# azrael417/mlperf-deepcam

Measured on AMD Instinct MI355X. Metric: samples/sec (768x1152x16) train step, higher is better.
Workload: dtype bf16; 1 GPU; DeepLabV3+/Xception train step (fwd + weighted CE + bwd + LAMB), 768x1152x16, local_batch=8, bf16 activations / fp32 master weights, random-init seed 333; local_batch=8, global_batch=8, parallelism=dp1, optimizer=LAMB, hip_graph=False, launch_list_replay=False

## Files before the change

### mlperf-deepcam_amd/csrc/common.h

```cpp
#pragma once
#include <hip/hip_runtime.h>
#include <stdint.h>

#include <mutex>

#include "../../include/deepcam_hip.h"

namespace dc {

typedef __bf16 bf16;
typedef __attribute__((ext_vector_type(8))) __bf16 bf16x8;
typedef __attribute__((ext_vector_type(4))) __bf16 bf16x4;
typedef __attribute__((ext_vector_type(4))) short short4v;
typedef __attribute__((ext_vector_type(4))) float f32x4;
typedef __attribute__((ext_vector_type(2))) float f32x2;

struct alignas(16) vec16 {
  uint32_t w[4];
};

template <typename T>
struct Elem;
template <>
struct Elem<float> {
  static constexpr int kPerVec = 4;
  static constexpr int kDtype = DC_F32;
  __device__ static inline float load(const float* p) { return *p; }
  __device__ static inline void store(float* p, float v) { *p = v; }
};
template <>
struct Elem<bf16> {
  static constexpr int kPerVec = 8;
  static constexpr int kDtype = DC_BF16;
  __device__ static inline float load(const bf16* p) { return (float)*p; }
  __device__ static inline void store(bf16* p, float v) { *p = (bf16)v; }
};

__device__ inline void unpack(const vec16& v, float (&f)[4], float) {
#pragma unroll
  for (int i = 0; i < 4; ++i) f[i] = __uint_as_float(v.w[i]);
}
__device__ inline void unpack(const vec16& v, float (&f)[8], bf16) {
#pragma unroll
  for (int i = 0; i < 4; ++i) {
    f[2 * i] = __uint_as_float(v.w[i] << 16);
    f[2 * i + 1] = __uint_as_float(v.w[i] & 0xffff0000u);
  }
}
__device__ inline uint32_t pack2_bf16(float lo, float hi) {
  typedef __attribute__((ext_vector_type(2))) __bf16 bf16x2;
  bf16x2 r;
  r[0] = (bf16)lo;
  r[1] = (bf16)hi;
  return __builtin_bit_cast(uint32_t, r);
}
__device__ inline void pack(vec16& v, const float (&f)[4], float) {
#pragma unroll
  for (int i = 0; i < 4; ++i) v.w[i] = __float_as_uint(f[i]);
}
__device__ inline void pack(vec16& v, const float (&f)[8], bf16) {
#pragma unroll
  for (int i = 0; i < 4; ++i) v.w[i] = pack2_bf16(f[2 * i], f[2 * i + 1]);
}

__device__ inline vec16 zero16() {
  vec16 z;
  z.w[0] = z.w[1] = z.w[2] = z.w[3] = 0u;
  return z;
}
__device__ inline vec16 ldg16(const void* p) { return *reinterpret_cast<const vec16*>(p); }
__device__ inline void stg16(void* p, const vec16& v) { *reinterpret_cast<vec16*>(p) = v; }

__device__ inline float wave_sum(float v) {
#pragma unroll
  for (int o = 32; o > 0; o >>= 1) v += __shfl_xor(v, o, 64);
  return v;
}
__device__ inline double wave_sum(double v) {
#pragma unroll
  for (int o = 32; o > 0; o >>= 1) v += __shfl_xor(v, o, 64);
  return v;
}

inline int cdiv(long a, long b) { return (int)((a + b - 1) / b); }

struct Options {
  int igemm256 = 1;
  int igemm256p = 1;
  int igemm256p_wgs = 0;
  int igemm256p_min = 257;
  int igemm256_splitk = 1;
  int pw384 = 1;
  int pw224 = 1;
  int pw192 = 1;
  int thin_tile = 1;
  int wgrad384 = 1;
  int wgrad384_slots = 192;
  int wgrad384_min_stages = 96;
  int head_fused = 1;
  int head_dgrad_fused = 1;
  int head_wgrad_fused = 1;
  int dw_tile = 1;
  int dw_wgrad_tpb = 0;
  int dw_pipe = 1;
  int bn_apply_rows = 1;
};
extern Options g_options;

const void* zero_page(hipError_t* err);

}

#define DC_ONCE(...)                               \
  do {                                             \
    static std::once_flag once_flag__;             \
    std::call_once(once_flag__, [&] { __VA_ARGS__; }); \
  } while (0)

namespace dc {
extern thread_local bool g_launch_log_on;
void launch_log_note(const char* name);
}

#define DC_LAUNCHED(name)                                  \
  do {                                                     \
    hipError_t e__ = hipGetLastError();                    \
    if (e__ != hipSuccess) return dc_set_error(e__, __FILE__, __LINE__); \
    if (dc::g_launch_log_on) dc::launch_log_note(name);    \
  } while (0)
#define DC_CHECK_LAUNCH() DC_LAUNCHED("aux")

extern "C" int dc_set_error(int code, const char* file, int line);
extern "C" int dc_fail(const char* msg, const char* file, int line);
extern "C" int dc_check_view(const void* ptr, int ld, int c, int dtype, const char* what);
#define DC_REQUIRE(cond, msg)                                  \
  do {                                                         \
    if (!(cond)) return dc_fail(msg, __FILE__, __LINE__);      \
  } while (0)
```

### mlperf-deepcam_amd/csrc/dwtile.hip

```cpp
#include "common.h"
#include "dwtile.h"
#include "dwtile_common.h"
#include "bn_fin.h"
#include "mfma_tile.h"

namespace dc {

constexpr int DT_TH = 8;

template <int DIL, int CG>
struct TileCfg {
  static constexpr int TH = DT_TH, TW = 8 * (32 / CG);
  static constexpr int HH = TH + 2 * DIL, HW = TW + 2 * DIL, HP = HH * HW;
  static constexpr int ITER = (HP * CG + 255) / 256;
  static constexpr int LDS_BYTES = ITER * 256 * 16;
  static constexpr int NSL = 128 / CG;
  static constexpr int SPR = TW / DT_PX;
  static constexpr int SPT = TH * SPR / NSL;
  static_assert(SPT * NSL == TH * SPR, "tile does not divide into strips");
};

static __device__ __attribute__((aligned(256))) unsigned char dwt_zero_page[256];

template <typename T, int DIL, int CG>
__device__ inline void stage_halo(char* smem, const T* __restrict__ in, int ldin, int n, int y0, int x0, int cg0, int ngroups, int H,
                                  int W) {
  typedef TileCfg<DIL, CG> K;
  constexpr int KPV = Elem<T>::kPerVec;
  const int tid = threadIdx.x;
  const int wv = __builtin_amdgcn_readfirstlane(tid >> 6);
  const int g = tid % CG;
  const bool gok = cg0 + g < ngroups;
  const T* base = in + (size_t)n * H * W * ldin + (size_t)(cg0 + g) * KPV;
#pragma unroll
  for (int it = 0; it < K::ITER; ++it) {
    const int hp = (it * 256 + tid) / CG;
    const int hy = hp / K::HW, hx = hp - hy * K::HW;
    const int iy = y0 - DIL + hy, ix = x0 - DIL + hx;
    const bool ok = gok && hp < K::HP && (unsigned)iy < (unsigned)H && (unsigned)ix < (unsigned)W;
    const void* src = ok ? (const void*)(base + ((size_t)iy * W + ix) * ldin) : (const void*)dwt_zero_page;
    __builtin_amdgcn_global_load_lds((gas_ptr)src, (lds_ptr)(smem + (it * 256 + wv * 64) * 16), 16, 0, 0);
  }
}

template <typename T, int DIL, bool FLIP, int CG, bool WG = false, int FIN = 0>
__global__ __launch_bounds__(256) void dwt_kernel(const T* __restrict__ in, int ldin, const float* __restrict__ wp,
                                                  const T* __restrict__ addend, int ldadd, T* __restrict__ out, int ldout, int H, int W,
                                                  int C, int ncgb, int ntx, int nty, const float* __restrict__ pscale,
                                                  const float* __restrict__ pshift, int prelu, const DwBnStats st, const BnFinArgs fin) {
  typedef TileCfg<DIL, CG> K;
  constexpr int KPV = Elem<T>::kPerVec, KH = KPV / 2;
  constexpr int WC = DT_PX + 2 * DIL;
  extern __shared__ __attribute__((aligned(16))) char smem[];
  const int t = xcd_remap(blockIdx.x, gridDim.x);
  const int cgb = t % ncgb;
  const int tile_id = t / ncgb;
  int r = t / ncgb;
  const int tx = r % ntx;
  r /= ntx;
  const int ty = r % nty, n = r / nty;
  const int ngroups = C / KPV;
  const int cg0 = cgb * CG, y0 = ty * K::TH, x0 = tx * K::TW;
  stage_halo<T, DIL, CG>(smem, in, ldin, n, y0, x0, cg0, ngroups, H, W);

  const int h = threadIdx.x % (2 * CG), sl = threadIdx.x / (2 * CG);
  const bool cok = cg0 + (h >> 1) < ngroups;
  const int ch0 = cok ? cg0 * KPV + h * KH : 0;
  float wk[9][KH];
  load_taps<KH>(wp, ch0, C, FLIP, wk);
  const float* ps = pscale;
  const float* psh = pshift;
  int cbase = 0;
  float fsc = 0.f, fsh = 0.f;
  if constexpr (FIN == 2) {
    constexpr int CW = CG * KPV;
    if (threadIdx.x < CW) {
      const int c = cg0 * KPV + threadIdx.x;
      if (c < C) {
        double s, q;
        sum_row_load(fin.slab, C, c, s, q);
        bn_fin_coefs(fin, c, s, q, tile_id == 0, fsc, fsh);
      }
    }
    if (t == 0 && threadIdx.x == 0 && fin.nbt != nullptr) *fin.nbt += 1;
  }
  if constexpr (FIN == 1) {
    constexpr int CW = CG * KPV;
    __shared__ float fincoef[2][CW];
    __shared__ double finred[2][4][CW];
    {
      double s, q;
      slab_quad_sum2<CW>(fin.slab, fin.rows, C, cg0 * KPV, finred, s, q);
      if (threadIdx.x < CW) {
        const int c = cg0 * KPV + threadIdx.x;
        float sc = 0.f, sh = 0.f;
        if (c < C) bn_fin_coefs(fin, c, s, q, tile_id == 0, sc, sh);
        fincoef[0][threadIdx.x] = sc;
        fincoef[1][threadIdx.x] = sh;
      }
      if (t == 0 && threadIdx.x == 0 && fin.nbt != nullptr) *fin.nbt += 1;
      ps = fincoef[0];
      psh = fincoef[1];
      cbase = cg0 * KPV;
    }
  }
  __syncthreads();
  if constexpr (FIN == 2) {
    constexpr int CW = CG * KPV;
    constexpr bool SLACK = K::LDS_BYTES - K::HP * CG * 16 >= 2 * CW * (int)sizeof(float);
    float* coef;
    if constexpr (SLACK) {
      coef = reinterpret_cast<float*>(smem + K::LDS_BYTES) - 2 * CW;
    } else {
      __shared__ float fincoef2[2 * CW];
      coef = fincoef2;
    }
    if (threadIdx.x < CW) {
      coef[threadIdx.x] = fsc;
      coef[CW + threadIdx.x] = fsh;
    }
    __syncthreads();
    ps = coef;
    psh = coef + CW;
    cbase = cg0 * KPV;
  }
  if (!FLIP && ps != nullptr) {
    bn_transform_tile<T, K::HH, K::HW, CG>(smem, y0 - DIL, x0 - DIL, H, W, ps, psh, prelu, cg0, ngroups, cbase);
    __syncthreads();
  }
  const bool stats = FLIP && st.slab != nullptr;
  if (!cok && !stats && !WG) return;
  BnAcc<KH> bn;
  if (stats) bn.init(st, ch0);
  else if (WG) bn.init_affine(st, ch0);
  float dwa[WG ? 9 : 1][KH];
  if constexpr (WG) {
#pragma unroll
    for (int t9 = 0; t9 < 9; ++t9)
#pragma unroll
      for (int e = 0; e < KH; ++e) dwa[t9][e] = 0.f;
  }

  const char* tile = smem + h * 8;
#pragma unroll 1
  for (int k = 0; k < (cok ? K::SPT : 0); ++k) {
    const int q = sl + K::NSL * k;
    const int row = q / K::SPR, xs = (q % K::SPR) * DT_PX;
    const int oy = y0 + row;
    vec8 yv[DT_PX];
    if (stats || WG) {
#pragma unroll
      for (int j = 0; j < DT_PX; ++j) {
        const int ox = x0 + xs + j;
        vec8 z;
        z.w[0] = z.w[1] = 0u;
        yv[j] = (oy < H && ox < W) ? *reinterpret_cast<const vec8*>(reinterpret_cast<const T*>(st.y) + (((size_t)n * H + oy) * W + ox) * st.ldy + ch0) : z;
      }
    }
    vec8 av[DT_PX];
    if (FLIP && addend != nullptr) {
#pragma unroll
      for (int j = 0; j < DT_PX; ++j) {
        const int ox = x0 + xs + j;
        vec8 z;
        z.w[0] = z.w[1] = 0u;
        av[j] = (oy < H && ox < W) ? *reinterpret_cast<const vec8*>(addend + (((size_t)n * H + oy) * W + ox) * ldadd + ch0) : z;
      }
    }
    float acc[DT_PX][KH];
#pragma unroll
    for (int j = 0; j < DT_PX; ++j)
#pragma unroll
      for (int e = 0; e < KH; ++e) acc[j][e] = 0.f;
    float xh[WG ? DT_PX : 1][KH];
    if constexpr (WG) {
#pragma unroll
      for (int j = 0; j < DT_PX; ++j) {
        const bool in = oy < H && x0 + xs + j < W;
        float yf[KH];
        unpack8(yv[j], yf, T());
#pragma unroll
        for (int e = 0; e < KH; ++e) {
          const float v = fmaf(yf[e], bn.ms[e], bn.mh[e]);
          yf[e] = st.relu ? fmaxf(v, 0.f) : v;
        }
        vec8 r;
        pack8(r, yf, T());
        unpack8(r, xh[j], T());
        if (!in) {
#pragma unroll
          for (int e = 0; e < KH; ++e) xh[j][e] = 0.f;
        }
      }
    }
#pragma unroll
    for (int ky = 0; ky < 3; ++ky) {
#pragma unroll
      for (int c = 0; c < WC; ++c) {
        float f[KH];
        unpack8(*reinterpret_cast<const vec8*>(tile + ((row + ky * DIL) * K::HW + xs + c) * (CG * 16)), f, T());
#pragma unroll
        for (int kx = 0; kx < 3; ++kx) {
          const int j = c - kx * DIL;
          if (j >= 0 && j < DT_PX) {
#pragma unroll
            for (int e = 0; e < KH; ++e) acc[j][e] = fmaf(f[e], wk[ky * 3 + kx][e], acc[j][e]);
            if constexpr (WG) {
#pragma unroll
              for (int e = 0; e < KH; ++e) dwa[8 - (ky * 3 + kx)][e] = fmaf(f[e], xh[j][e], dwa[8 - (ky * 3 + kx)][e]);
            }
          }
        }
      }
    }
    if (oy < H) {
#pragma unroll
      for (int j = 0; j < DT_PX; ++j) {
        const int ox = x0 + xs + j;
        if (ox < W) {
          const size_t opix = ((size_t)n * H + oy) * W + ox;
          if (FLIP && addend != nullptr) {
            float a[KH];
            unpack8(av[j], a, T());
#pragma unroll
            for (int e = 0; e < KH; ++e) acc[j][e] += a[e];
          }
          vec8 v;
          pack8(v, acc[j], T());
          *reinterpret_cast<vec8*>(out + opix * ldout + ch0) = v;
          if (stats) {
            float gs[KH], yf[KH];
            unpack8(v, gs, T());
            unpack8(yv[j], yf, T());
            bn.add(gs, yf, st.relu);
          }
        }
      }
    }
  }
  if (stats) {
    __syncthreads();
    bn_acc_store<KH, K::NSL, CG * KPV>(reinterpret_cast<float*>(smem), bn.a, bn.b, cok, h, sl, st, tile_id, cg0 * KPV, C);
  }
  if constexpr (WG) {
    __syncthreads();
    float* red = reinterpret_cast<float*>(smem);
    constexpr int CW = CG * KPV;
    if (cok) {
#pragma unroll
      for (int tp = 0; tp < 9; ++tp)
#pragma unroll
        for (int e = 0; e < KH; ++e) red[(sl * 9 + tp) * CW + h * KH + e] = dwa[tp][e];
    }
    __syncthreads();
    for (int i = threadIdx.x; i < 9 * CW; i += 256) {
      const int tp = i / CW, cl = i % CW;
      const int c = cg0 * KPV + cl;
      if (c < C) {
        float sacc = 0.f;
#pragma unroll
        for (int qq = 0; qq < K::NSL; ++qq) sacc += red[(qq * 9 + tp) * CW + cl];
        st.wslab[((size_t)tile_id * 9 + tp) * C + c] = sacc;
      }
    }
  }
}

template <typename T, int DIL, int CG>
__global__ __launch_bounds__(256) void dwt_wgrad_kernel(const T* __restrict__ x, int ldx, const T* __restrict__ dy, int lddy,
                                                        float* __restrict__ slab, int H, int W, int C, int ncgb, int ntx, int nty,
                                                        int ntiles, int tpb, const float* __restrict__ pscale,
                                                        const float* __restrict__ pshift, int prelu) {
  typedef TileCfg<DIL, CG> K;
  constexpr int KPV = Elem<T>::kPerVec, KH = KPV / 2;
  constexpr int WC = DT_PX + 2 * DIL;
  extern __shared__ __attribute__((aligned(16))) char smem[];
  const int t = xcd_remap(blockIdx.x, gridDim.x);
  const int cgb = t % ncgb, srow = t / ncgb;
  const int ngroups = C / KPV;
  const int cg0 = cgb * CG;
  const int h = threadIdx.x % (2 * CG), sl = threadIdx.x / (2 * CG);
  const bool cok = cg0 + (h >> 1) < ngroups;
  const int ch0 = cok ? cg0 * KPV + h * KH : 0;
  float acc[9][KH];
#pragma unroll
  for (int tp = 0; tp < 9; ++tp)
#pragma unroll
    for (int e = 0; e < KH; ++e) acc[tp][e] = 0.f;

  const int tbeg = srow * tpb, tend = min(ntiles, tbeg + tpb);
  const char* tile = smem + h * 8;
  for (int ti = tbeg; ti < tend; ++ti) {
    const int tx = ti % ntx;
    int r = ti / ntx;
    const int ty = r % nty, n = r / nty;
    const int y0 = ty * K::TH, x0 = tx * K::TW;
    if (ti != tbeg) __syncthreads();
    stage_halo<T, DIL, CG>(smem, x, ldx, n, y0, x0, cg0, ngroups, H, W);
    auto load_dy = [&](int k, vec8 (&gv)[DT_PX]) {
      const int q = sl + K::NSL * k;
      const int row = q / K::SPR, xs = (q % K::SPR) * DT_PX;
      const int oy = y0 + row;
#pragma unroll
      for (int j = 0; j < DT_PX; ++j) {
        const int ox = x0 + xs + j;
        const bool ok = cok && oy < H && ox < W;
        vec8 z;
        z.w[0] = z.w[1] = 0u;
        gv[j] = ok ? *reinterpret_cast<const vec8*>(dy + (((size_t)n * H + oy) * W + ox) * lddy + ch0) : z;
      }
    };
    vec8 gcur[DT_PX], gnext[DT_PX];
    load_dy(0, gcur);
    __syncthreads();
    if (pscale != nullptr) {
      bn_transform_tile<T, K::HH, K::HW, CG>(smem, y0 - DIL, x0 - DIL, H, W, pscale, pshift, prelu, cg0, ngroups);
      __syncthreads();
    }
    if (cok) {
#pragma unroll 1
      for (int k = 0; k < K::SPT; ++k) {
        if (k + 1 < K::SPT) load_dy(k + 1, gnext);
        const int q = sl + K::NSL * k;
        const int row = q / K::SPR, xs = (q % K::SPR) * DT_PX;
        float gf[DT_PX][KH];
#pragma unroll
        for (int j = 0; j < DT_PX; ++j) unpack8(gcur[j], gf[j], T());
#pragma unroll
        for (int ky = 0; ky < 3; ++ky)
#pragma unroll
          for (int c = 0; c < WC; ++c) {
            float f[KH];
            unpack8(*reinterpret_cast<const vec8*>(tile + ((row + ky * DIL) * K::HW + xs + c) * (CG * 16)), f, T());
#pragma unroll
            for (int kx = 0; kx < 3; ++kx) {
              const int j = c - kx * DIL;
              if (j >= 0 && j < DT_PX) {
#pragma unroll
                for (int e = 0; e < KH; ++e) acc[ky * 3 + kx][e] = fmaf(gf[j][e], f[e], acc[ky * 3 + kx][e]);
              }
            }
          }
#pragma unroll
        for (int j = 0; j < DT_PX; ++j) gcur[j] = gnext[j];
      }
    }
  }
  __syncthreads();
  float* red = reinterpret_cast<float*>(smem);
  constexpr int CW = CG * KPV;
#pragma unroll
  for (int tp = 0; tp < 9; ++tp)
#pragma unroll
    for (int e = 0; e < KH; ++e) red[(sl * 9 + tp) * CW + h * KH + e] = acc[tp][e];
  __syncthreads();
  for (int i = threadIdx.x; i < 9 * CW; i += 256) {
    const int tp = i / CW, cl = i % CW;
    const int c = cg0 * KPV + cl;
    if (c < C) {
      float s = 0.f;
#pragma unroll
      for (int q = 0; q < K::NSL; ++q) s += red[(q * 9 + tp) * CW + cl];
      slab[((size_t)srow * 9 + tp) * C + c] = s;
    }
  }
}

__global__ __launch_bounds__(256) void dwt_reduce_kernel(const float* __restrict__ slab, float* __restrict__ grad, int rows, int C) {
  __shared__ double red[16][16];
  const int cl = threadIdx.x & 15, rl = threadIdx.x >> 4;
  const int n = 9 * C;
  const int i = blockIdx.x * 16 + cl;
  double a0 = 0.0, a1 = 0.0;
  if (i < n) {
    int r = rl;
    for (; r + 16 < rows; r += 32) {
      a0 += (double)slab[(size_t)r * n + i];
      a1 += (double)slab[(size_t)(r + 16) * n + i];
    }
    if (r < rows) a0 += (double)slab[(size_t)r * n + i];
  }
  red[rl][cl] = a0 + a1;
  __syncthreads();
  if (threadIdx.x < 16 && blockIdx.x * 16 + threadIdx.x < n) {
    const int j = blockIdx.x * 16 + threadIdx.x;
    double s = 0.0;
#pragma unroll
    for (int k = 0; k < 16; ++k) s += red[k][threadIdx.x];
    const int tp = j / C, c = j % C;
    grad[(size_t)c * 9 + tp] = (float)s;
  }
}

int dw_tile_reduce(const float* slab, float* grad_w, int rows, int C, hipStream_t st) {
  hipLaunchKernelGGL(dwt_reduce_kernel, dim3(cdiv(9 * C, 16)), dim3(256), 0, st, slab, grad_w, rows, C);
  DC_LAUNCHED("dw_tile_reduce");
  return 0;
}

static int pick_cg(int ngroups) { return ngroups <= 8 ? 8 : ngroups <= 16 ? 16 : 32; }

struct TileGrid {
  int cg, ncgb, ntx, nty, ntiles;
};
static TileGrid tile_grid(int ngroups, int N, int H, int W) {
  TileGrid t;
  t.cg = pick_cg(ngroups);
  const int tw = 8 * (32 / t.cg);
  t.ncgb = cdiv(ngroups, t.cg);
  t.ntx = cdiv(W, tw);
  t.nty = cdiv(H, DT_TH);
  t.ntiles = N * t.ntx * t.nty;
  return t;
}

static int wgrad_tpb(const TileGrid& t) {
  if (g_options.dw_wgrad_tpb > 0) return g_options.dw_wgrad_tpb;
  long tpb = ((long)t.ntiles * t.ncgb + 256) / 512;
  if (tpb < 1) tpb = 1;
  while (cdiv(t.ntiles, tpb) > DWT_MAX_ROWS) ++tpb;
  return (int)tpb;
}

int dw_tile_rows(int dtype, int C, int N, int H, int W) { return tile_grid(C / (dtype == DC_BF16 ? 8 : 4), N, H, W).ntiles; }

size_t dw_tile_wgrad_workspace(int C, int N, int H, int W) {
  size_t best = 0;
  for (int kpv = 4; kpv <= 8; kpv += 4) {
    if (C % kpv) continue;
    const TileGrid t = tile_grid(C / kpv, N, H, W);
    const int rows = t.ntiles < DWT_MAX_ROWS ? t.ntiles : DWT_MAX_ROWS;
    const size_t b = (size_t)rows * 9 * C * sizeof(float);
    if (b > best) best = b;
  }
  return best;
}

template <typename T, int DIL, bool FLIP, int CG>
static void launch_fwd1(const TileGrid& t, const void* in, int ldin, const float* wp, const void* addend, int ldadd, void* out,
                        int ldout, int H, int W, int C, hipStream_t st, const float* pscale, const float* pshift, int prelu, const DwBnStats& bs, const BnFinArgs& fin) {
  if constexpr (FLIP) {
    if (bs.wslab != nullptr) {
      constexpr int FOLD = TileCfg<DIL, CG>::NSL * 9 * CG * Elem<T>::kPerVec * (int)sizeof(float);
      constexpr int LDSW = TileCfg<DIL, CG>::LDS_BYTES > FOLD ? TileCfg<DIL, CG>::LDS_BYTES : FOLD;
      DC_ONCE((void)hipFuncSetAttribute(reinterpret_cast<const void*>(&dwt_kernel<T, DIL, true, CG, true>), hipFuncAttributeMaxDynamicSharedMemorySize, LDSW));
      hipLaunchKernelGGL((dwt_kernel<T, DIL, true, CG, true>), dim3(t.ntiles * t.ncgb), dim3(256), LDSW, st, (const T*)in, ldin, wp,
                         (const T*)addend, ldadd, (T*)out, ldout, H, W, C, t.ncgb, t.ntx, t.nty, pscale, pshift, prelu, bs, fin);
      return;
    }
  }
  constexpr int LDS = TileCfg<DIL, CG>::LDS_BYTES;
  if constexpr (!FLIP) {
    if (fin.slab != nullptr && fin.rows == SUM_ROW) {
      DC_ONCE((void)hipFuncSetAttribute(reinterpret_cast<const void*>(&dwt_kernel<T, DIL, false, CG, false, 2>), hipFuncAttributeMaxDynamicSharedMemorySize, LDS));
      hipLaunchKernelGGL((dwt_kernel<T, DIL, false, CG, false, 2>), dim3(t.ntiles * t.ncgb), dim3(256), LDS, st, (const T*)in, ldin, wp,
                         (const T*)addend, ldadd, (T*)out, ldout, H, W, C, t.ncgb, t.ntx, t.nty, pscale, pshift, prelu, bs, fin);
      return;
    }
    if (fin.slab != nullptr) {
      DC_ONCE((void)hipFuncSetAttribute(reinterpret_cast<const void*>(&dwt_kernel<T, DIL, false, CG, false, 1>), hipFuncAttributeMaxDynamicSharedMemorySize, LDS));
      hipLaunchKernelGGL((dwt_kernel<T, DIL, false, CG, false, 1>), dim3(t.ntiles * t.ncgb), dim3(256), LDS, st, (const T*)in, ldin, wp,
                         (const T*)addend, ldadd, (T*)out, ldout, H, W, C, t.ncgb, t.ntx, t.nty, pscale, pshift, prelu, bs, fin);
      return;
    }
  }
  DC_ONCE((void)hipFuncSetAttribute(reinterpret_cast<const void*>(&dwt_kernel<T, DIL, FLIP, CG>), hipFuncAttributeMaxDynamicSharedMemorySize, LDS));
  hipLaunchKernelGGL((dwt_kernel<T, DIL, FLIP, CG>), dim3(t.ntiles * t.ncgb), dim3(256), LDS, st, (const T*)in, ldin, wp,
                     (const T*)addend, ldadd, (T*)out, ldout, H, W, C, t.ncgb, t.ntx, t.nty, pscale, pshift, prelu, bs, fin);
}

template <typename T, int DIL, bool FLIP>
static void launch_fwd2(const TileGrid& t, const void* in, int ldin, const float* wp, const void* addend, int ldadd, void* out,
                        int ldout, int H, int W, int C, hipStream_t st, const float* pscale, const float* pshift, int prelu, const DwBnStats& bs, const BnFinArgs& fin) {
  if (t.cg == 32) launch_fwd1<T, DIL, FLIP, 32>(t, in, ldin, wp, addend, ldadd, out, ldout, H, W, C, st, pscale, pshift, prelu, bs, fin);
  else if (t.cg == 16) launch_fwd1<T, DIL, FLIP, 16>(t, in, ldin, wp, addend, ldadd, out, ldout, H, W, C, st, pscale, pshift, prelu, bs, fin);
  else launch_fwd1<T, DIL, FLIP, 8>(t, in, ldin, wp, addend, ldadd, out, ldout, H, W, C, st, pscale, pshift, prelu, bs, fin);
}

int launch_dw_tile(int dtype, int dil, bool flip, const void* in, int ldin, const float* wp, const void* addend, int ldadd,
                   void* out, int ldout, int N, int H, int W, int C, hipStream_t st, const float* pscale, const float* pshift, int prelu,
                   const DwBnStats* bnstats, const BnFinArgs* finp) {
  const int kpv = dtype == DC_BF16 ? 8 : 4;
  BnFinArgs fin;
  if (finp != nullptr) fin = *finp; else fin.slab = nullptr;
  DC_REQUIRE(finp == nullptr || (!flip && !dw_pipe_forward() && finp->rows <= FIN_RL && finp->parts == 0),
             "dc_dwconv_fwd_fin: a forward pass on the tiled kernel over a slab of at most dc_bn_bwd_apply_fin_max_rows() rows");
  if ((flip || dw_pipe_forward()) && (long)N * H * W < (1L << 31) && dw_pipe_rows(dtype, C, dil, N, H, W) > 0)
    return launch_dw_pipe(dil, flip, in, ldin, wp, addend, ldadd, out, ldout, N, H, W, C, st, pscale, pshift, prelu, bnstats);
  DC_REQUIRE(bnstats == nullptr || bnstats->rows != SUM_ROW, "dc_dwconv_dgrad_*_sum: a sum row is served by the pipelined kernel only (dc_dwconv_dgrad_sum_row_ok)");
  const TileGrid t = tile_grid(C / kpv, N, H, W);
  DC_REQUIRE((long)t.ntiles * t.ncgb < (1L << 31) && (long)N * H * W < (1L << 31), "dc_dwconv: tensor too large for the tiled path");
  DwBnStats bs;
  if (bnstats != nullptr) bs = *bnstats; else { bs.slab = nullptr; bs.y = nullptr; bs.ldy = 0; bs.mean = bs.invstd = bs.mscale = bs.mshift = nullptr; bs.relu = 0; bs.rows = 0; bs.wslab = nullptr; }
  if (bs.slab != nullptr) bs.rows = t.ntiles;
#define DWT(TT, D, F) launch_fwd2<TT, D, F>(t, in, ldin, wp, addend, ldadd, out, ldout, H, W, C, st, pscale, pshift, prelu, bs, fin)
  if (dtype == DC_BF16) {
    if (dil == 1) { if (flip) DWT(bf16, 1, true); else DWT(bf16, 1, false); }
    else          { if (flip) DWT(bf16, 2, true); else DWT(bf16, 2, false); }
  } else {
    if (dil == 1) { if (flip) DWT(float, 1, true); else DWT(float, 1, false); }
    else          { if (flip) DWT(float, 2, true); else DWT(float, 2, false); }
  }
#undef DWT
  DC_LAUNCHED(flip ? "dw_tile_dgrad" : "dw_tile_fwd");
  return 0;
}

template <typename T, int DIL, int CG>
static void launch_wg1(const TileGrid& t, int tpb, int rows, const void* x, int ldx, const void* dy, int lddy, float* slab, int H,
                       int W, int C, hipStream_t st, const float* pscale, const float* pshift, int prelu) {
  constexpr int FOLD = TileCfg<DIL, CG>::NSL * 9 * CG * Elem<T>::kPerVec * (int)sizeof(float);
  constexpr int LDS = TileCfg<DIL, CG>::LDS_BYTES > FOLD ? TileCfg<DIL, CG>::LDS_BYTES : FOLD;
  DC_ONCE((void)hipFuncSetAttribute(reinterpret_cast<const void*>(&dwt_wgrad_kernel<T, DIL, CG>), hipFuncAttributeMaxDynamicSharedMemorySize, LDS));
  hipLaunchKernelGGL((dwt_wgrad_kernel<T, DIL, CG>), dim3(rows * t.ncgb), dim3(256), LDS, st, (const T*)x, ldx, (const T*)dy, lddy,
                     slab, H, W, C, t.ncgb, t.ntx, t.nty, t.ntiles, tpb, pscale, pshift, prelu);
}

template <typename T, int DIL>
static void launch_wg2(const TileGrid& t, int tpb, int rows, const void* x, int ldx, const void* dy, int lddy, float* slab, int H,
                       int W, int C, hipStream_t st, const float* pscale, const float* pshift, int prelu) {
  if (t.cg == 32) launch_wg1<T, DIL, 32>(t, tpb, rows, x, ldx, dy, lddy, slab, H, W, C, st, pscale, pshift, prelu);
  else if (t.cg == 16) launch_wg1<T, DIL, 16>(t, tpb, rows, x, ldx, dy, lddy, slab, H, W, C, st, pscale, pshift, prelu);
  else launch_wg1<T, DIL, 8>(t, tpb, rows, x, ldx, dy, lddy, slab, H, W, C, st, pscale, pshift, prelu);
}

int launch_dw_tile_wgrad(int dtype, int dil, const void* x, int ldx, const void* dy, int lddy, float* slab, float* grad_w, int N,
                         int H, int W, int C, hipStream_t st, const float* pscale, const float* pshift, int prelu) {
  const int kpv = dtype == DC_BF16 ? 8 : 4;
  const TileGrid t = tile_grid(C / kpv, N, H, W);
  const int tpb = wgrad_tpb(t);
  const int rows = cdiv(t.ntiles, tpb);
  DC_REQUIRE(rows <= DWT_MAX_ROWS, "dc_dwconv_wgrad: tiles-per-workgroup override needs more slab rows than the workspace holds");
  DC_REQUIRE((long)N * H * W < (1L << 31), "dc_dwconv_wgrad: tensor too large for the tiled path");
  if (dtype == DC_BF16) {
    if (dil == 1) launch_wg2<bf16, 1>(t, tpb, rows, x, ldx, dy, lddy, slab, H, W, C, st, pscale, pshift, prelu);
    else launch_wg2<bf16, 2>(t, tpb, rows, x, ldx, dy, lddy, slab, H, W, C, st, pscale, pshift, prelu);
  } else {
    if (dil == 1) launch_wg2<float, 1>(t, tpb, rows, x, ldx, dy, lddy, slab, H, W, C, st, pscale, pshift, prelu);
    else launch_wg2<float, 2>(t, tpb, rows, x, ldx, dy, lddy, slab, H, W, C, st, pscale, pshift, prelu);
  }
  DC_LAUNCHED("dw_tile_wgrad");
  hipLaunchKernelGGL(dwt_reduce_kernel, dim3(cdiv(9 * C, 16)), dim3(256), 0, st, (const float*)slab, grad_w, rows, C);
  DC_LAUNCHED("dw_tile_reduce");
  return 0;
}

}
```

### mlperf-deepcam_amd/csrc/dwtile_common.h

```cpp
#pragma once
#include "common.h"

namespace dc {

constexpr int DT_PX = 4;

__device__ inline int xcd_remap(int bid, int nwg) {
  const int q8 = nwg >> 3, r8 = nwg & 7, xcd = bid & 7, slot = bid >> 3;
  return (xcd < r8 ? xcd * (q8 + 1) : r8 * (q8 + 1) + (xcd - r8) * q8) + slot;
}

struct alignas(8) vec8 {
  uint32_t w[2];
};
__device__ inline void unpack8(const vec8& v, float (&f)[2], float) {
  f[0] = __uint_as_float(v.w[0]);
  f[1] = __uint_as_float(v.w[1]);
}
__device__ inline void unpack8(const vec8& v, float (&f)[4], bf16) {
#pragma unroll
  for (int i = 0; i < 2; ++i) {
    f[2 * i] = __uint_as_float(v.w[i] << 16);
    f[2 * i + 1] = __uint_as_float(v.w[i] & 0xffff0000u);
  }
}
__device__ inline void pack8(vec8& v, const float (&f)[2], float) {
  v.w[0] = __float_as_uint(f[0]);
  v.w[1] = __float_as_uint(f[1]);
}
__device__ inline void pack8(vec8& v, const float (&f)[4], bf16) {
  v.w[0] = pack2_bf16(f[0], f[1]);
  v.w[1] = pack2_bf16(f[2], f[3]);
}

template <int KH>
__device__ inline void load_taps(const float* __restrict__ wp, int ch0, int C, bool flip, float (&wk)[9][KH]) {
#pragma unroll
  for (int t = 0; t < 9; ++t) {
    const float* src = wp + (size_t)(flip ? 8 - t : t) * C + ch0;
    if constexpr (KH == 4) {
      const float4 v = *reinterpret_cast<const float4*>(src);
      wk[t][0] = v.x; wk[t][1] = v.y; wk[t][2] = v.z; wk[t][3] = v.w;
    } else {
      const float2 v = *reinterpret_cast<const float2*>(src);
      wk[t][0] = v.x; wk[t][1] = v.y;
    }
  }
}


struct DwBnStats {
  const void* y;
  int ldy;
  const float* mean;
  const float* invstd;
  const float* mscale;
  const float* mshift;
  int relu;
  float* slab;
  int rows;
  float* wslab;
};

template <int KH>
struct BnAcc {
  float mu[KH], is[KH], ms[KH], mh[KH], a[KH], b[KH];
  __device__ inline void init(const DwBnStats& st, int ch0) {
    const bool affine = st.relu || st.wslab != nullptr;
#pragma unroll
    for (int e = 0; e < KH; ++e) {
      mu[e] = st.mean[ch0 + e];
      is[e] = st.invstd[ch0 + e];
      ms[e] = affine ? st.mscale[ch0 + e] : 0.f;
      mh[e] = affine ? st.mshift[ch0 + e] : 0.f;
      a[e] = b[e] = 0.f;
    }
  }
  __device__ inline void init_affine(const DwBnStats& st, int ch0) {
#pragma unroll
    for (int e = 0; e < KH; ++e) {
      mu[e] = is[e] = a[e] = b[e] = 0.f;
      ms[e] = st.mscale != nullptr ? st.mscale[ch0 + e] : 1.f;
      mh[e] = st.mshift != nullptr ? st.mshift[ch0 + e] : 0.f;
    }
  }
  __device__ inline void add(const float (&g)[KH], const float (&yv)[KH], int relu) {
#pragma unroll
    for (int e = 0; e < KH; ++e) {
      const float gm = (!relu || fmaf(yv[e], ms[e], mh[e]) > 0.f) ? g[e] : 0.f;
      a[e] += gm;
      b[e] = fmaf(gm, (yv[e] - mu[e]) * is[e], b[e]);
    }
  }
};

template <int KH, int NSL, int CW>
__device__ inline void bn_acc_store(float* red, const float (&a)[KH], const float (&b)[KH], bool cok, int h, int sl, const DwBnStats& st,
                                    int tile, int c_base, int C) {
  if (cok) {
#pragma unroll
    for (int e = 0; e < KH; ++e) {
      red[(sl * 2 + 0) * CW + h * KH + e] = a[e];
      red[(sl * 2 + 1) * CW + h * KH + e] = b[e];
    }
  }
  __syncthreads();
  for (int i = threadIdx.x; i < 2 * CW; i += 256) {
    const int which = i / CW, cl = i % CW;
    if (c_base + cl < C) {
      float s = 0.f;
#pragma unroll
      for (int q = 0; q < NSL; ++q) s += red[(q * 2 + which) * CW + cl];
      st.slab[((size_t)which * st.rows + tile) * C + c_base + cl] = s;
    }
  }
}

template <typename T, int HH, int HW, int CG>
__device__ inline void bn_transform_tile(char* smem, int iy0, int ix0, int H, int W, const float* __restrict__ pscale,
                                         const float* __restrict__ pshift, int prelu, int cg0, int ngroups, int cbase = 0) {
  constexpr int KPV = Elem<T>::kPerVec;
  constexpr int HP = HH * HW, ITER = (HP * CG + 255) / 256;
  const int tid = threadIdx.x, g = tid % CG;
  if (cg0 + g >= ngroups) return;
  float sc[KPV], sh[KPV];
#pragma unroll
  for (int e = 0; e < KPV; ++e) {
    sc[e] = pscale[(cg0 + g) * KPV + e - cbase];
    sh[e] = pshift[(cg0 + g) * KPV + e - cbase];
  }
#pragma unroll 2
  for (int it = 0; it < ITER; ++it) {
    const int slot = it * 256 + tid;
    const int hp = slot / CG;
    const int hy = hp / HW, hx = hp - hy * HW;
    const int iy = iy0 + hy, ix = ix0 + hx;
    if (hp < HP && (unsigned)iy < (unsigned)H && (unsigned)ix < (unsigned)W) {
      vec16* q = reinterpret_cast<vec16*>(smem) + slot;
      float f[KPV];
      unpack(*q, f, T());
#pragma unroll
      for (int e = 0; e < KPV; ++e) {
        const float v = fmaf(f[e], sc[e], sh[e]);
        f[e] = prelu ? fmaxf(v, 0.f) : v;
      }
      vec16 o;
      pack(o, f, T());
      *q = o;
    }
  }
}

}
```

### mlperf-deepcam_amd/csrc/igemm.hip

```cpp
#include <stdio.h>
#include <string.h>

#include <type_traits>

#include "conv_geom.h"
#include "igemm.h"
#include "mfma_tile.h"

namespace dc {

constexpr int BM = 128, BN = 128;
constexpr int ROWB = 64, NSTAGE = 3;

template <typename T>
struct Mma;
template <>
struct Mma<bf16> {
  __device__ static inline void run(const vec16& a, const vec16& b, f32x4& c) {
    c = __builtin_amdgcn_mfma_f32_16x16x32_bf16(__builtin_bit_cast(bf16x8, a), __builtin_bit_cast(bf16x8, b), c, 0, 0, 0);
  }
};
template <>
struct Mma<float> {
  __device__ static inline void run(const vec16& a, const vec16& b, f32x4& c) {
// ... 593 lines not shown
}

__device__ inline void pack_pointwise_tile_bf16(const PackEntry& e, int tile, float* lds) {
  const int A = e.kind == 1 ? e.cin : e.cout, B = e.kind == 1 ? e.cout : e.cin;
  bf16* P = reinterpret_cast<bf16*>(e.kind == 1 ? e.wb : e.wf);
  bf16* Q = reinterpret_cast<bf16*>(e.kind == 1 ? e.wf : e.wb);
  const int ldp = weight_ld(B), ldq = weight_ld(A);
  constexpr int TS = 64, ROWF = TS + 1;
  const int ntb = (B + TS - 1) / TS;
  const int a0 = (tile / ntb) * TS, b0 = (tile % ntb) * TS;
  const int run = min(TS, B - b0);
  __syncthreads();
#pragma unroll
  for (int idx = threadIdx.x; idx < TS * (TS / 4); idx += 256) {
    const int al = idx / (TS / 4), j = (idx % (TS / 4)) * 4;
    float4 v = make_float4(0.f, 0.f, 0.f, 0.f);
    if (a0 + al < A && j < run) v = *reinterpret_cast<const float4*>(e.master + (size_t)(a0 + al) * B + b0 + j);
    float* d = lds + al * ROWF + j;
    d[0] = v.x; d[1] = v.y; d[2] = v.z; d[3] = v.w;
  }
  __syncthreads();
  if (P != nullptr) {
#pragma unroll
    for (int idx = threadIdx.x; idx < TS * (TS / 8); idx += 256) {
      const int u = idx % (TS / 8), al = idx / (TS / 8);
      if (a0 + al < A && b0 + u * 8 < B) {
        float f[8];
#pragma unroll
        for (int k = 0; k < 8; ++k) f[k] = lds[al * ROWF + u * 8 + k];
        vec16 v;
        pack(v, f, bf16());
        stg16(P + (size_t)(a0 + al) * ldp + b0 + u * 8, v);
      }
    }
  }
  if (Q != nullptr) {
#pragma unroll
    for (int idx = threadIdx.x; idx < TS * (TS / 8); idx += 256) {
      const int u = idx % (TS / 8), bl = idx / (TS / 8);
      if (b0 + bl < B && a0 + u * 8 < A) {
        float f[8];
#pragma unroll
        for (int k = 0; k < 8; ++k) f[k] = lds[(u * 8 + k) * ROWF + bl];
        vec16 v;
        pack(v, f, bf16());
        stg16(Q + (size_t)(b0 + bl) * ldq + a0 + u * 8, v);
      }
    }
  }
}

__device__ inline int pack_entry_tiles(const PackEntry& e) {
  if (e.kind == 2) return (e.cout + 255) / 256;
  const int A = e.kind == 1 ? e.cin : e.cout, B = e.kind == 1 ? e.cout : e.cin;
  const int TS = e.taps == 1 ? 64 : 32;
  return ((A + TS - 1) / TS) * ((B + TS - 1) / TS);
}

constexpr int PACK_MAX_ENTRIES = 1024;

template <typename T>
__global__ __launch_bounds__(256) void pack_all_kernel(const PackEntry* __restrict__ table, int nentries) {
  __shared__ float lds[sizeof(T) == 2 ? PACK_LDS_FLOATS_BF16 : PACK_LDS_FLOATS];
  __shared__ int prefix[PACK_MAX_ENTRIES + 1];
  for (int i = threadIdx.x; i < nentries; i += 256) prefix[i + 1] = pack_entry_tiles(table[i]);
  if (threadIdx.x == 0) prefix[0] = 0;
  __syncthreads();
  if (threadIdx.x == 0)
    for (int i = 1; i <= nentries; ++i) prefix[i] += prefix[i - 1];
  __syncthreads();
  const int total = prefix[nentries];
  for (int gt = blockIdx.x; gt < total; gt += gridDim.x) {
    int lo = 0, hi = nentries;
    while (hi - lo > 1) {
      const int mid = (lo + hi) >> 1;
      if (prefix[mid] <= gt) lo = mid; else hi = mid;
    }
    const PackEntry e = table[lo];
    const int tile = gt - prefix[lo];
    if (e.kind == 2) {
      float* out = reinterpret_cast<float*>(e.wf);
      const int c = tile * 256 + threadIdx.x;
      if (c < e.cout) {
#pragma unroll
        for (int t = 0; t < 9; ++t) out[(size_t)t * e.cout + c] = e.master[(size_t)c * 9 + t];
      }
      continue;
    }
    if (e.taps == 1) {
      if constexpr (sizeof(T) == 2) {
        if (((e.cin | e.cout) & 7) == 0) pack_pointwise_tile_bf16(e, tile, lds);
        else pack_dense_tile<T, 1>(e, tile, lds);
      } else {
        pack_dense_tile<T, 1>(e, tile, lds);
      }
    } else {
      pack_dense_tile<T, 9>(e, tile, lds);
    }
  }
}

}

using namespace dc;

constexpr int PACK_BLOCKS = 2048;
extern "C" int dc_pack_all(int dtype, const void* table_dev, int nentries, void* stream) {
  DC_REQUIRE(table_dev != nullptr && nentries > 0, "dc_pack_all: bad argument");
  DC_REQUIRE(sizeof(PackEntry) == 40, "dc_pack_all: entry layout changed");
  DC_REQUIRE(nentries <= PACK_MAX_ENTRIES, "dc_pack_all: too many entries for one launch");
  dim3 grid(PACK_BLOCKS);
  if (dtype == DC_BF16) hipLaunchKernelGGL(pack_all_kernel<bf16>, grid, dim3(256), 0, (hipStream_t)stream, (const PackEntry*)table_dev, nentries);
  else hipLaunchKernelGGL(pack_all_kernel<float>, grid, dim3(256), 0, (hipStream_t)stream, (const PackEntry*)table_dev, nentries);
  DC_CHECK_LAUNCH();
  return 0;
}

Options dc::g_options;

static __device__ __attribute__((aligned(256))) unsigned char dc_arg_zero_page[256];

const void* dc::zero_page(hipError_t* err) {
  static void* dev = nullptr;
  static hipError_t init_err = hipSuccess;
  DC_ONCE({ init_err = hipGetSymbolAddress(&dev, HIP_SYMBOL(dc_arg_zero_page)); });
  *err = init_err;
  return dev;
}

namespace {
enum class Norm { kValue, kFlag, kZeroToTwo, kNonNegative, kPositive, kStages };
const struct {
  const char* name;
  int Options::*field;
  Norm norm;
} kOptions[] = {
    {"igemm256", &Options::igemm256, Norm::kValue},
    {"igemm256p", &Options::igemm256p, Norm::kValue},
    {"igemm256p_wgs", &Options::igemm256p_wgs, Norm::kValue},
    {"igemm256p_min", &Options::igemm256p_min, Norm::kValue},
    {"igemm256_splitk", &Options::igemm256_splitk, Norm::kValue},
    {"pw384", &Options::pw384, Norm::kValue},
    {"pw224", &Options::pw224, Norm::kValue},
    {"pw192", &Options::pw192, Norm::kValue},
    {"thin_tile", &Options::thin_tile, Norm::kFlag},
    {"wgrad384", &Options::wgrad384, Norm::kValue},
    {"wgrad384_slots", &Options::wgrad384_slots, Norm::kPositive},
    {"wgrad384_min_stages", &Options::wgrad384_min_stages, Norm::kStages},
    {"head_fused", &Options::head_fused, Norm::kFlag},
    {"head_dgrad_fused", &Options::head_dgrad_fused, Norm::kFlag},
    {"head_wgrad_fused", &Options::head_wgrad_fused, Norm::kFlag},
    {"dw_tile", &Options::dw_tile, Norm::kFlag},
    {"dw_wgrad_tpb", &Options::dw_wgrad_tpb, Norm::kNonNegative},
    {"dw_pipe", &Options::dw_pipe, Norm::kZeroToTwo},
    {"bn_apply_rows", &Options::bn_apply_rows, Norm::kFlag},
};
}

extern "C" int dc_set_option(const char* name, int value) {
  for (const auto& o : kOptions) {
    if (name == nullptr || strcmp(name, o.name) != 0) continue;
    switch (o.norm) {
      case Norm::kValue: break;
      case Norm::kFlag: value = value != 0; break;
      case Norm::kZeroToTwo: value = value < 0 ? 0 : value > 2 ? 2 : value; break;
      case Norm::kNonNegative: value = value < 0 ? 0 : value; break;
      case Norm::kPositive:
      case Norm::kStages:
        if (value < 1) {
          char msg[96];
          snprintf(msg, sizeof(msg), "dc_set_option: %s must be positive", o.name);
          return dc_fail(msg, __FILE__, __LINE__);
        }
        if (o.norm == Norm::kStages && value < 4) value = 4;
        break;
    }
    g_options.*o.field = value;
    return 0;
  }
  return dc_fail("dc_set_option: unknown option", __FILE__, __LINE__);
}

extern "C" int dc_reset_options(void) {
  g_options = Options{};
  return 0;
}

extern "C" int dc_conv_out_hw(const dc_conv_desc* d, int Hi, int Wi, int* Ho, int* Wo) {
  DC_REQUIRE(d != nullptr, "dc_conv_out_hw: null descriptor");
  GatherGeom g;
  if (!build_geom(*d, Hi, Wi, kFwd, &g)) return dc_fail("dc_conv_out_hw: unsupported geometry", __FILE__, __LINE__);
  if (Ho) *Ho = g.Hout;
  if (Wo) *Wo = g.Wout;
  return 0;
}

extern "C" int dc_conv_stat_rows(const dc_conv_desc* d, int N, int Hi, int Wi) {
  GatherGeom g;
  if (d == nullptr || !build_geom(*d, Hi, Wi, kFwd, &g)) return -1;
  return cdiv((long)N * g.Qh * g.Qw, BM) * g.os * g.os;
}

extern "C" int dc_conv_fwd(const dc_conv_desc* d, int N, int Hi, int Wi, const void* x, int ldx, const void* wf,
                           const float* bias, void* y, int ldy, float* stat_slab, int accumulate, void* stream) {
  return run_gather(d, kFwd, N, Hi, Wi, x, ldx, wf, bias, y, ldy, stat_slab, accumulate, stream);
}

extern "C" int dc_conv_fwd_kn(const dc_conv_desc* d, int N, int Hi, int Wi, const void* x, int ldx, const void* wf, const void* wb,
                              const float* bias, void* y, int ldy, float* stat_slab, int slab_rows, int accumulate, void* stream) {
  return run_gather(d, kFwd, N, Hi, Wi, x, ldx, wf, bias, y, ldy, stat_slab, accumulate, stream, false, nullptr, wb, slab_rows);
}
static int kn_forward_plan(const dc_conv_desc* d, int N, int Hi, int Wi, long* Mout) {
  const int plain = dc_conv_stat_rows(d, N, Hi, Wi);
  if (plain <= 0 || d->dtype != DC_BF16) return 0;
  IgemmParams p;
  if (!build_geom(*d, Hi, Wi, kFwd, &p.g)) return 0;
  const long M = (long)N * p.g.Qh * p.g.Qw;
  if (M >= (1L << 31) - BM) return 0;
  if (M <= TINY_M || thin_fwd_eligible(p.g, d->dtype, false, 0, false)) return 0;
  p.x = nullptr; p.w = nullptr; p.y = nullptr; p.bias = nullptr; p.slab = nullptr;
  p.N = N; p.ldx = weight_ld(p.g.Cin); p.ldy = weight_ld(p.g.Cout); p.ldw = weight_ld(p.g.Cin);
  alignas(16) static const char some_image[16] = {0};
  p.w_kn = some_image;
  p.ldw_kn = weight_ld(p.g.Cout);
  p.M = (int)M;
  p.mtiles = cdiv(M, BM);
  *Mout = M;
  return pw384_plan(p);
}
extern "C" int dc_conv_stat_rows_kn(const dc_conv_desc* d, int N, int Hi, int Wi) {
  long M = 0;
  const int npb = kn_forward_plan(d, N, Hi, Wi, &M);
  return (npb == 224 || npb == 226) ? cdiv(M, 224) : dc_conv_stat_rows(d, N, Hi, Wi);
}
extern "C" int dc_conv_sum_row_kn(const dc_conv_desc* d, int N, int Hi, int Wi) {
  if (d == nullptr) return 0;
  long M = 0;
  const int npb = kn_forward_plan(d, N, Hi, Wi, &M);
  return npb == 224 || npb == 226 || npb == 192 ? 1 : 0;
}
extern "C" int dc_conv_dgrad_kn(const dc_conv_desc* d, int N, int Hi, int Wi, const void* dy, int lddy, const void* wb, const void* wf,
                                void* dx, int lddx, int accumulate, void* stream) {
  return run_gather(d, kDgrad, N, Hi, Wi, dy, lddy, wb, nullptr, dx, lddx, nullptr, accumulate, stream, false, nullptr, wf);
}

static int dilated_group_impl(const dc_conv_desc* d, int N, int Hi, int Wi, int count, const int* dils, const void* x, int ldx,
                              const void* const* wfs, void* const* ys, int ldy, float* const* stat_slabs, void* ws, size_t ws_bytes,
                              size_t* want_bytes, void* stream) {
  DC_REQUIRE(d != nullptr && dils != nullptr && (want_bytes != nullptr || (wfs != nullptr && ys != nullptr)), "dc_conv_fwd_dilated_group: null argument");
  DC_REQUIRE(count >= 1 && count <= IgemmParams::MAXGROUP, "dc_conv_fwd_dilated_group: count must be 1..4");
  DC_REQUIRE(!d->transposed && d->k == 3 && d->stride == 1, "dc_conv_fwd_dilated_group: 3x3, stride 1 convolutions only");
  if (want_bytes != nullptr) *want_bytes = 0;
  for (int b = 0; b < count; ++b) DC_REQUIRE(dils[b] >= 1 && (want_bytes != nullptr || (wfs[b] != nullptr && ys[b] != nullptr)), "dc_conv_fwd_dilated_group: bad member");
  const bool fused = count > 1 && d->dtype == DC_BF16 && g_options.igemm256 != 0;
  if (!fused) {
    if (want_bytes != nullptr) return 0;
    for (int b = 0; b < count; ++b) {
      dc_conv_desc db = *d;
      db.dil = db.pad = dils[b];
      if (int e = run_gather(&db, kFwd, N, Hi, Wi, x, ldx, wfs[b], nullptr, ys[b], ldy, stat_slabs ? stat_slabs[b] : nullptr, 0, stream)) return e;
    }
    return 0;
  }
  dc_conv_desc du = *d;
  du.dil = du.pad = 1;
  IgemmParams p;
  if (!build_geom(du, Hi, Wi, kFwd, &p.g)) return dc_fail("dc_conv_fwd_dilated_group: unsupported geometry", __FILE__, __LINE__);
  if (want_bytes == nullptr) {
    if (int e = check_view(x, ldx, p.g.Cin, d->dtype, "dc_conv_fwd_dilated_group input")) return e;
    for (int b = 0; b < count; ++b) {
      if (int e = check_view(ys[b], ldy, p.g.Cout, d->dtype, "dc_conv_fwd_dilated_group output")) return e;
      DC_REQUIRE(((uintptr_t)wfs[b] & 15) == 0, "dc_conv_fwd_dilated_group: weights unaligned");
    }
  }
  const long M = (long)N * p.g.Qh * p.g.Qw;
  DC_REQUIRE(N > 0 && M < (1L << 31) - BM, "dc_conv_fwd_dilated_group: bad pixel count");
  p.x = x; p.w = wfs ? wfs[0] : nullptr; p.y = ys ? ys[0] : nullptr; p.bias = nullptr; p.slab = stat_slabs ? stat_slabs[0] : nullptr;
  p.N = N; p.ldx = ldx; p.ldy = ldy;
  p.ldw = weight_ld(p.g.Cin);
  p.M = (int)M;
  p.mtiles = cdiv(M, BM);
  p.ngroup = count;
  size_t need = 0;
  const int splits = igemm256_splitk_plan(p, &need);
  if (want_bytes != nullptr) {
    *want_bytes = need;
    return 0;
  }
  for (int b = 0; b < IgemmParams::MAXGROUP; ++b) p.gdil[b] = b < count ? dils[b] : 1;
  for (int b = 1; b < IgemmParams::MAXGROUP; ++b) {
    p.gw[b - 1] = b < count ? wfs[b] : nullptr;
    p.gy[b - 1] = b < count ? ys[b] : nullptr;
    p.gslab[b - 1] = (b < count && stat_slabs) ? stat_slabs[b] : nullptr;
  }
  if (stat_slabs)
    for (int b = 0; b < count; ++b) DC_REQUIRE(stat_slabs[b] != nullptr, "dc_conv_fwd_dilated_group: statistics for all members or none");
  if (splits > 1 && ws != nullptr && ws_bytes >= need) {
    DC_REQUIRE(((uintptr_t)ws & 15) == 0, "dc_conv_fwd_dilated_group_ws: workspace unaligned");
    return launch_igemm256_splitk(p, splits, ws, (hipStream_t)stream);
  }
  return launch_igemm256(p, (hipStream_t)stream);
}

extern "C" int dc_conv_fwd_dilated_group(const dc_conv_desc* d, int N, int Hi, int Wi, int count, const int* dils, const void* x,
                                         int ldx, const void* const* wfs, void* const* ys, int ldy, float* const* stat_slabs,
                                         void* stream) {
// ... 62 lines not shown
```

Before: 261.4 samples/s.

## Add row-blocked depthwise forward kernel with register sliding window over rows

Adds a specialized depthwise 3x3 forward kernel for the non-flipped path. Each thread computes a 4-row by strip block, walking input rows once and accumulating into all output rows that use them, so each LDS value is read once rather than reloaded per tap row. It also adds an unrolled BN-apply-on-tile variant with the ReLU branch resolved at compile time and cheaper index arithmetic. It is on by default through a new option flag and drops the addend and stats paths from this kernel, which raises register use per thread.

```diff
diff --git a/mlperf-deepcam_amd/csrc/common.h b/mlperf-deepcam_amd/csrc/common.h
--- a/mlperf-deepcam_amd/csrc/common.h
+++ b/mlperf-deepcam_amd/csrc/common.h
@@ -102,6 +102,7 @@
   int head_wgrad_fused = 1;
   int dw_tile = 1;
   int dw_wgrad_tpb = 0;
+  int dw_fwd_rows = 1;
   int dw_pipe = 1;
   int bn_apply_rows = 1;
 };
diff --git a/mlperf-deepcam_amd/csrc/dwtile.hip b/mlperf-deepcam_amd/csrc/dwtile.hip
--- a/mlperf-deepcam_amd/csrc/dwtile.hip
+++ b/mlperf-deepcam_amd/csrc/dwtile.hip
@@ -40,6 +40,59 @@
     const bool ok = gok && hp < K::HP && (unsigned)iy < (unsigned)H && (unsigned)ix < (unsigned)W;
     const void* src = ok ? (const void*)(base + ((size_t)iy * W + ix) * ldin) : (const void*)dwt_zero_page;
     __builtin_amdgcn_global_load_lds((gas_ptr)src, (lds_ptr)(smem + (it * 256 + wv * 64) * 16), 16, 0, 0);
+  }
+}
+
+constexpr int DT_ROWS = 4;
+template <typename T, int DIL, int CG, int KH>
+__device__ __forceinline__ void dwt_rows_tile(const char* __restrict__ tile, const float (&wk)[9][KH], int r0, int xs, int y0, int x0, int n, int H,
+                                              int W, T* __restrict__ out, int ldout) {
+  typedef TileCfg<DIL, CG> K;
+  static_assert(2 * DT_ROWS == K::TH && 2 * K::SPR == K::NSL, "two row halves x the column strips = the strip lanes");
+  constexpr int WR = DT_ROWS + 2 * DIL, WC = DT_PX + 2 * DIL;
+  float acc[DT_ROWS][DT_PX][KH];
+#pragma unroll
+  for (int o = 0; o < DT_ROWS; ++o)
+#pragma unroll
+    for (int j = 0; j < DT_PX; ++j)
+#pragma unroll
+      for (int e = 0; e < KH; ++e) acc[o][j][e] = 0.f;
+#pragma unroll
+  for (int ii = 0; ii < WR; ++ii) {
+    const int i = DIL == 1 ? ii : ii / (WR / DIL) + (ii % (WR / DIL)) * DIL;
+#pragma unroll
+    for (int c = 0; c < WC; ++c) {
+      float f[KH];
+      unpack8(*reinterpret_cast<const vec8*>(tile + ((r0 + i) * K::HW + xs + c) * (CG * 16)), f, T());
+#pragma unroll
+      for (int ky = 0; ky < 3; ++ky) {
+        const int o = i - ky * DIL;
+        if (o < 0 || o >= DT_ROWS) continue;
+#pragma unroll
+        for (int kx = 0; kx < 3; ++kx) {
+          const int j = c - kx * DIL;
+          if (j >= 0 && j < DT_PX) {
+#pragma unroll
+            for (int e = 0; e < KH; ++e) acc[o][j][e] = fmaf(f[e], wk[ky * 3 + kx][e], acc[o][j][e]);
+          }
+        }
+      }
+    }
+    const int od = i - 2 * DIL;
+    if (od >= 0) {
+      const int oy = y0 + r0 + od;
+      if (oy < H) {
+#pragma unroll
+        for (int j = 0; j < DT_PX; ++j) {
+          const int ox = x0 + xs + j;
+          if (ox < W) {
+            vec8 r;
+            pack8(r, acc[od][j], T());
+            *reinterpret_cast<vec8*>(out + (((size_t)n * H + oy) * W + ox) * ldout) = r;
+          }
+        }
+      }
+    }
   }
 }
 
@@ -266,6 +319,94 @@
   }
 }
 
+template <typename T, int DIL, int CG, int FIN>
+__global__ __launch_bounds__(256) void dwt_rows_kernel(const T* __restrict__ in, int ldin, const float* __restrict__ wp, T* __restrict__ out,
+                                                       int ldout, int H, int W, int C, int ncgb, int ntx, int nty,
+                                                       const float* __restrict__ pscale, const float* __restrict__ pshift, int prelu,
+                                                       const BnFinArgs fin) {
+  typedef TileCfg<DIL, CG> K;
+  constexpr int KPV = Elem<T>::kPerVec, KH = KPV / 2;
+  extern __shared__ __attribute__((aligned(16))) char smem[];
+  const int t = xcd_remap(blockIdx.x, gridDim.x);
+  const int cgb = t % ncgb;
+  const int tile_id = t / ncgb;
+  int r = t / ncgb;
+  const int tx = r % ntx;
+  r /= ntx;
+  const int ty = r % nty, n = r / nty;
+  const int ngroups = C / KPV;
+  const int cg0 = cgb * CG, y0 = ty * K::TH, x0 = tx * K::TW;
+  stage_halo<T, DIL, CG>(smem, in, ldin, n, y0, x0, cg0, ngroups, H, W);
+
+  const int h = threadIdx.x % (2 * CG), sl = threadIdx.x / (2 * CG);
+  const bool cok = cg0 + (h >> 1) < ngroups;
+  const int ch0 = cok ? cg0 * KPV + h * KH : 0;
+  float wk[9][KH];
+  load_taps<KH>(wp, ch0, C, false, wk);
+  const float* ps = pscale;
+  const float* psh = pshift;
+  int cbase = 0;
+  float fsc = 0.f, fsh = 0.f;
+  if constexpr (FIN == 2) {
+    constexpr int CW = CG * KPV;
+    if (threadIdx.x < CW) {
+      const int c = cg0 * KPV + threadIdx.x;
+      if (c < C) {
+        double s, q;
+        sum_row_load(fin.slab, C, c, s, q);
+        bn_fin_coefs(fin, c, s, q, tile_id == 0, fsc, fsh);
+      }
+    }
+    if (t == 0 && threadIdx.x == 0 && fin.nbt != nullptr) *fin.nbt += 1;
+  }
+  if constexpr (FIN == 1) {
+    constexpr int CW = CG * KPV;
+    __shared__ float fincoef[2][CW];
+    __shared__ double finred[2][4][CW];
+    double s, q;
+    slab_quad_sum2<CW>(fin.slab, fin.rows, C, cg0 * KPV, finred, s, q);
+    if (threadIdx.x < CW) {
+      const int c = cg0 * KPV + threadIdx.x;
+      float sc = 0.f, sh = 0.f;
+      if (c < C) bn_fin_coefs(fin, c, s, q, tile_id == 0, sc, sh);
+      fincoef[0][threadIdx.x] = sc;
+      fincoef[1][threadIdx.x] = sh;
+    }
+    if (t == 0 && threadIdx.x == 0 && fin.nbt != nullptr) *fin.nbt += 1;
+    ps = fincoef[0];
+    psh = fincoef[1];
+    cbase = cg0 * KPV;
+  }
+  __syncthreads();
+  if constexpr (FIN == 2) {
+    constexpr int CW = CG * KPV;
+    constexpr bool SLACK = K::LDS_BYTES - K::HP * CG * 16 >= 2 * CW * (int)sizeof(float);
+    float* coef;
+    if constexpr (SLACK) {
+      coef = reinterpret_cast<float*>(smem + K::LDS_BYTES) - 2 * CW;
+    } else {
+      __shared__ float fincoef2[2 * CW];
+      coef = fincoef2;
+    }
+    if (threadIdx.x < CW) {
+      coef[threadIdx.x] = fsc;
+      coef[CW + threadIdx.x] = fsh;
+    }
+    __syncthreads();
+    ps = coef;
+    psh = coef + CW;
+    cbase = cg0 * KPV;
+  }
+  const int r0 = (sl / K::SPR) * DT_ROWS, xs = (sl % K::SPR) * DT_PX;
+  if (FIN != 0 || ps != nullptr) {
+    if (prelu) bn_transform_tile_u<T, K::HH, K::HW, CG, true>(smem, y0 - DIL, x0 - DIL, H, W, ps, psh, cg0, ngroups, cbase);
+    else bn_transform_tile_u<T, K::HH, K::HW, CG, false>(smem, y0 - DIL, x0 - DIL, H, W, ps, psh, cg0, ngroups, cbase);
+    __syncthreads();
+  }
+  if (!cok || y0 + r0 >= H) return;
+  dwt_rows_tile<T, DIL, CG>(smem + h * 8, wk, r0, xs, y0, x0, n, H, W, out + ch0, ldout);
+}
+
 template <typename T, int DIL, int CG>
 __global__ __launch_bounds__(256) void dwt_wgrad_kernel(const T* __restrict__ x, int ldx, const T* __restrict__ dy, int lddy,
                                                         float* __restrict__ slab, int H, int W, int C, int ncgb, int ntx, int nty,
@@ -436,6 +577,15 @@
   return best;
 }
 
+template <typename T, int DIL, int CG, int FIN>
+static void launch_fwd_rows(const TileGrid& t, const void* in, int ldin, const float* wp, void* out, int ldout, int H, int W, int C, hipStream_t st,
+                            const float* pscale, const float* pshift, int prelu, const BnFinArgs& fin) {
+  constexpr int LDS = TileCfg<DIL, CG>::LDS_BYTES;
+  DC_ONCE((void)hipFuncSetAttribute(reinterpret_cast<const void*>(&dwt_rows_kernel<T, DIL, CG, FIN>), hipFuncAttributeMaxDynamicSharedMemorySize, LDS));
+  hipLaunchKernelGGL((dwt_rows_kernel<T, DIL, CG, FIN>), dim3(t.ntiles * t.ncgb), dim3(256), LDS, st, (const T*)in, ldin, wp, (T*)out, ldout, H, W, C,
+                     t.ncgb, t.ntx, t.nty, pscale, pshift, prelu, fin);
+}
+
 template <typename T, int DIL, bool FLIP, int CG>
 static void launch_fwd1(const TileGrid& t, const void* in, int ldin, const float* wp, const void* addend, int ldadd, void* out,
                         int ldout, int H, int W, int C, hipStream_t st, const float* pscale, const float* pshift, int prelu, const DwBnStats& bs, const BnFinArgs& fin) {
@@ -451,6 +601,12 @@
   }
   constexpr int LDS = TileCfg<DIL, CG>::LDS_BYTES;
   if constexpr (!FLIP) {
+    if (g_options.dw_fwd_rows) {
+      if (fin.slab == nullptr) launch_fwd_rows<T, DIL, CG, 0>(t, in, ldin, wp, out, ldout, H, W, C, st, pscale, pshift, prelu, fin);
+      else if (fin.rows == SUM_ROW) launch_fwd_rows<T, DIL, CG, 2>(t, in, ldin, wp, out, ldout, H, W, C, st, pscale, pshift, prelu, fin);
+      else launch_fwd_rows<T, DIL, CG, 1>(t, in, ldin, wp, out, ldout, H, W, C, st, pscale, pshift, prelu, fin);
+      return;
+    }
     if (fin.slab != nullptr && fin.rows == SUM_ROW) {
       DC_ONCE((void)hipFuncSetAttribute(reinterpret_cast<const void*>(&dwt_kernel<T, DIL, false, CG, false, 2>), hipFuncAttributeMaxDynamicSharedMemorySize, LDS));
       hipLaunchKernelGGL((dwt_kernel<T, DIL, false, CG, false, 2>), dim3(t.ntiles * t.ncgb), dim3(256), LDS, st, (const T*)in, ldin, wp,
diff --git a/mlperf-deepcam_amd/csrc/dwtile_common.h b/mlperf-deepcam_amd/csrc/dwtile_common.h
--- a/mlperf-deepcam_amd/csrc/dwtile_common.h
+++ b/mlperf-deepcam_amd/csrc/dwtile_common.h
@@ -151,4 +151,41 @@
   }
 }
 
+template <typename T, int HH, int HW, int CG, bool RELU>
+__device__ __forceinline__ void bn_transform_tile_u(char* smem, int iy0, int ix0, int H, int W, const float* __restrict__ pscale,
+                                                    const float* __restrict__ pshift, int cg0, int ngroups, int cbase) {
+  constexpr int KPV = Elem<T>::kPerVec;
+  constexpr int HP = HH * HW, ITER = (HP * CG + 255) / 256, PPI = 256 / CG;
+  const int tid = threadIdx.x, g = tid % CG;
+  if (cg0 + g >= ngroups) return;
+  float sc[KPV], sh[KPV];
+#pragma unroll
+  for (int e = 0; e < KPV; ++e) {
+    sc[e] = pscale[(cg0 + g) * KPV + e - cbase];
+    sh[e] = pshift[(cg0 + g) * KPV + e - cbase];
+  }
+  const int hp0 = tid / CG;
+  const int hy0 = hp0 / HW, hx0 = hp0 - hy0 * HW;
+  vec16* q0 = reinterpret_cast<vec16*>(smem) + tid;
+#pragma unroll
+  for (int it = 0; it < ITER; ++it) {
+    int hx = hx0 + (it * PPI) % HW, hy = hy0 + (it * PPI) / HW;
+    if (hx >= HW) { hx -= HW; ++hy; }
+    const int iy = iy0 + hy, ix = ix0 + hx;
+    if (hy < HH && (unsigned)iy < (unsigned)H && (unsigned)ix < (unsigned)W) {
+      vec16* q = q0 + it * 256;
+      float f[KPV];
+      unpack(*q, f, T());
+#pragma unroll
+      for (int e = 0; e < KPV; ++e) {
+        const float v = fmaf(f[e], sc[e], sh[e]);
+        f[e] = RELU ? fmaxf(v, 0.f) : v;
+      }
+      vec16 o;
+      pack(o, f, T());
+      *q = o;
+    }
+  }
 }
+
+}
diff --git a/mlperf-deepcam_amd/csrc/igemm.hip b/mlperf-deepcam_amd/csrc/igemm.hip
--- a/mlperf-deepcam_amd/csrc/igemm.hip
+++ b/mlperf-deepcam_amd/csrc/igemm.hip
@@ -769,6 +769,7 @@
     {"head_wgrad_fused", &Options::head_wgrad_fused, Norm::kFlag},
     {"dw_tile", &Options::dw_tile, Norm::kFlag},
     {"dw_wgrad_tpb", &Options::dw_wgrad_tpb, Norm::kNonNegative},
+    {"dw_fwd_rows", &Options::dw_fwd_rows, Norm::kFlag},
     {"dw_pipe", &Options::dw_pipe, Norm::kZeroToTwo},
     {"bn_apply_rows", &Options::bn_apply_rows, Norm::kFlag},
 };
```

Result: no change. 263.2 samples/s (median of 6 runs) (+0.7%).
